# huakunyang/SummerTTS

Measured on AMD Instinct MI355X. Metric: audio samples/sec (acoustic model + vocoder, phoneme ids -> int16 PCM on host), single_speaker_fast-shaped synthetic blob, higher is better.
Workload: dtype f32 (decoder trunk convs AND the reverse flow's WaveNet convs (wn_flow.hip, one-utterance calls): fp32 operands as 2 fp16 terms = 22-23 of their 24 mantissa bits, 3 fp16 MFMA products per fp32 product, f32 accumulation -- measured error in `parity`, same tolerance as the exact-fp32 leg; batches addi

## Files before the change

### include/summertts_hip.h

```cpp
#ifndef SUMMERTTS_HIP_H_
#define SUMMERTTS_HIP_H_

#include <stdint.h>

#ifdef __cplusplus
extern "C" {
#endif

typedef struct sts_engine sts_engine;

enum {
    STS_OK = 0,
    STS_EINVAL = -1,
    STS_EMODEL = -2,
    STS_EDEVICE = -3,
    STS_ESTATE = -4
};

int sts_create(const float* blob, int64_t blob_bytes, int device, sts_engine** out);
void sts_destroy(sts_engine* e);

int sts_speaker_num(const sts_engine* e);

typedef struct sts_model_info {
// ... 61 lines not shown

enum { STS_DBG_ATTN_BLOCK_MIN_WGS = 1,
       STS_DBG_TAIL_FUSED = 14 ,
       STS_DBG_UPS_ROWPH = 15 ,
       STS_DBG_CHAIN_STREAMS = 13 ,
       STS_DBG_H2P = 11 ,
       STS_DBG_H2P_TILE = 12 ,
       STS_DBG_MEMO_CLEAR = 10 ,
       STS_DBG_PCM_DIRECT = 9 ,
       STS_DBG_DDS_TAIL = 8 ,
       STS_DBG_ATTN_REG = 7 ,
       STS_DBG_LAUNCH_AHEAD = 6 ,
       STS_DBG_FLOW_FUSED = 5  };
enum { STS_DBG_STREAM_RETRY_STEP = 16, STS_DBG_STREAM_DIRECT = 17 };
enum { STS_DBG_POISON = 18 };
int sts_debug_set(sts_engine* e, int key, int value);

typedef struct sts_profile {
    float ms_text_encoder, ms_duration, ms_flow, ms_decoder, ms_total_device;
    float ms_decoder_mfma;
    int32_t decoder_mfma_launches;
    double flops_text_encoder, flops_duration, flops_flow, flops_decoder;
    double flops_decoder_mfma;
    double bytes_decoder_min;
    int64_t frames, samples, phonemes;
    double flops_decoder_mfma_executed;
    double bytes_text_encoder, bytes_duration, bytes_flow;
    float ms_sync_wait_host;
    double flops_decoder_bf16_issued;
    int64_t conv_math_fallbacks;
    int32_t conv_math_pinned;
    int32_t launch_ahead;
    int64_t launch_ahead_misses;
    float us_host_setup;
    float us_host_enqueue;
    float us_host_tail;
    int64_t poison_bytes;
} sts_profile;
int sts_set_profiling(sts_engine* e, int enable);
#define STS_ABI_VERSION 13
int sts_abi_version(void);
int sts_build_flags(void);
int sts_get_profile(const sts_engine* e, sts_profile* p);
int sts_get_profile_ex(const sts_engine* e, void* p, int64_t size_bytes);

int sts_debug_conv1d(int device, const float* x, int32_t Cin, int32_t L, const float* w, const float* bias,
                     int32_t Cout, int32_t k, int32_t pad, int32_t dil, int32_t stride_transposed,
                     int32_t depthwise, float in_slope, int32_t in_act, int mode, float** y, int32_t* Lout);

int sts_debug_conv1d_bench(int device, const float* x, int32_t Cin, int32_t L, const float* w, const float* bias,
                           int32_t Cout, int32_t k, int32_t pad, int32_t dil, int32_t stride_transposed,
                           int32_t depthwise, float in_slope, int32_t in_act, int mode, float** y, int32_t* Lout,
                           int32_t iters, float* ms_out);

int sts_debug_conv_h2p(int device, const float* x, int32_t Cin, int32_t L, const float* w, const float* bias, int32_t Cout, int32_t k,
// ... 53 lines not shown
```

### summertts_amd/csrc/capi.hip

```cpp
#include <stdlib.h>
#include <string.h>

#include <algorithm>
#include <new>
#include <string>
#include <vector>

#include "engine.hpp"

using namespace sts;

struct sts_engine { Engine eng; };

static thread_local std::string g_err;
static int set_err(int code, const std::string& s) { g_err = s; return code; }

extern "C" {

const char* sts_last_error(void) { return g_err.c_str(); }
void sts_free(void* p) { free(p); }

int sts_create(const float* blob, int64_t blob_bytes, int device, sts_engine** out) {
    if (!out) return set_err(STS_EINVAL, "sts_create: null out pointer");
    *out = nullptr;
// ... 157 lines not shown
        case STS_DBG_ATTN_BLOCK_MIN_WGS: if (value < 1) return set_err(STS_EINVAL, "threshold must be >= 1"); e->eng.attn_block_min_wgs = value; return STS_OK;
        case STS_DBG_FLOW_FUSED: e->eng.flow_fused = value != 0; return STS_OK;
        case STS_DBG_LAUNCH_AHEAD: if (value < 0 || value > 2) return set_err(STS_EINVAL, "launch_ahead must be 0, 1 or 2"); if ((value == 2) != (e->eng.launch_ahead == 2)) { e->eng.seen_tf_.clear(); e->eng.seen_order_.clear(); } e->eng.launch_ahead = value; return STS_OK;
        case STS_DBG_H2P: e->eng.h2p = value < 0 ? 0 : (value > 4 ? 4 : value); return STS_OK;
        case STS_DBG_H2P_TILE: e->eng.h2p_tile = value; return STS_OK;
        case STS_DBG_CHAIN_STREAMS: e->eng.chain_streams_dbg = value; return STS_OK;
        case STS_DBG_TAIL_FUSED: e->eng.tail_fused = value != 0; return STS_OK;
        case STS_DBG_UPS_ROWPH: e->eng.ups_rowph = value != 0; return STS_OK;
        case STS_DBG_MEMO_CLEAR: e->eng.seen_tf_.clear(); e->eng.seen_order_.clear(); return STS_OK;
        case STS_DBG_ATTN_REG: e->eng.attn_reg = value != 0; return STS_OK;
        case STS_DBG_DDS_TAIL: e->eng.dds_tail = value != 0; return STS_OK;
        case STS_DBG_PCM_DIRECT: e->eng.pcm_direct = value != 0; return STS_OK;
        case STS_DBG_STREAM_RETRY_STEP: e->eng.stream_retry_step = value < 0 ? -1 : value; return STS_OK;
        case STS_DBG_STREAM_DIRECT: e->eng.stream_direct = value != 0; return STS_OK;
        case STS_DBG_POISON: e->eng.poison = (unsigned)value; return STS_OK;
        default: return set_err(STS_EINVAL, "unknown debug key");
    }
}
int sts_set_host_pcm(sts_engine* e, int enable) { if (!e) return set_err(STS_EINVAL, "null engine"); e->eng.host_pcm = enable != 0; return STS_OK; }
int sts_set_profiling(sts_engine* e, int enable) { if (!e) return set_err(STS_EINVAL, "null engine"); e->eng.profiling = enable == 2 ? 2 : (enable != 0 ? 1 : 0); return STS_OK; }

int sts_abi_version(void) { return STS_ABI_VERSION; }

int sts_set_output_rate(sts_engine* e, int32_t rate) {
    if (!e) return set_err(STS_EINVAL, "null engine");
    const int rc = e->eng.set_output_rate(rate);
    return rc == STS_OK ? STS_OK : set_err(rc, e->eng.error());
}
int sts_get_output_rate(const sts_engine* e) {
    if (!e) return set_err(STS_EINVAL, "null engine");
// ... 489 lines not shown
```

### summertts_amd/csrc/conv_bf3.hip

```cpp
#include "conv_bf3_dev.hpp"

namespace sts {

#ifdef STS_TILE_TRACE
int tile_trace_bind_group(long long* buf, unsigned capacity_records);
int tile_trace_bind_resblock(long long* buf, unsigned capacity_records);
int tile_trace_bind_flow(long long* buf, unsigned capacity_records);
int tile_trace_bind_h2p(long long* buf, unsigned capacity_records);
static long long* g_tt_host_buf = nullptr;
extern "C" int sts_debug_tile_trace(long long* buf, unsigned capacity_records) {
    g_tt_host_buf = buf;
    if (buf && hipMemset(buf, 0, 16 * sizeof(long long)) != hipSuccess) return -1;
    if (tile_trace_bind(buf, capacity_records) || tile_trace_bind_group(buf, capacity_records) || tile_trace_bind_resblock(buf, capacity_records) || tile_trace_bind_flow(buf, capacity_records) || tile_trace_bind_h2p(buf, capacity_records)) return -1;
    return 0;
}
extern "C" int sts_debug_tile_trace_count() {
    unsigned n = 0;
    if (!g_tt_host_buf || hipMemcpy(&n, g_tt_host_buf, sizeof(unsigned), hipMemcpyDeviceToHost) != hipSuccess) return -1;
    return (int)n;
}
#endif

static inline void split_host(float x, uint16_t (&p)[3]) {
    uint32_t u; memcpy(&u, &x, 4);
// ... 55 lines not shown
    return bytes;
}

bool conv_bf3_eligible(const ConvArgs& a) {
    if (!a.wb3 || a.depthwise || (a.in_reflect && a.transposed)) return false;
    if (a.Cin != a.Cin_pad || a.Cin_pad % CK != 0 || a.Cout_pad % 32 != 0 || a.Cin < 32) return false;
    if ((double)a.x_ld * 64.0 >= 4.0e9) return false;
    const int first = a.tap_off, last = a.tap_off + (a.ntap - 1) * a.tap_step;
    const int halo = first < last ? last - first : first - last;
    if (halo > MAX_HALO) return false;
    if (a.epi == EPI_GATE && !a.gate_perm) return false;
    if (a.epi == EPI_TANH_PCM || a.kslices > 1) return false;
    return true;
}

template <int MW, int NW, int WM, int WN, int NSUB, int KG = 1, bool H2 = false, bool SUM = false>
static void launch_bf3(const ConvArgs& a, int nphase, hipStream_t st, int pm = 0) {
    constexpr int MT = 32 * MW * WM, NT = 32 * NW * WN;
    pm = pm && a.transposed && (MW == 1 || a.Cout_pad % (32 * MW) == 0);
    const int mt = pm ? (a.Cout_pad * nphase + MT - 1) / MT : (a.Cout_pad + MT - 1) / MT;
    const int nx = (a.max_n + NT - 1) / NT, ny = pm ? mt : mt * nphase;
    if constexpr (SUM) {
        if (a.nsum >= 2) {
            if (a.math == 1) {
                const size_t lds = bf3_lds_bytes<MW, NW, WM, WN, NSUB, KG, 1>();
                hipLaunchKernelGGL((conv_bf3_kernel<MW, NW, WM, WN, NSUB, KG, 1, true>), dim3(mapped_grid(nx, ny, a.B)), dim3(WM * WN * KG * 64), lds, st, a, mt, nx, ny, pm);
            } else {
                const size_t lds = bf3_lds_bytes<MW, NW, WM, WN, NSUB, KG>();
                hipLaunchKernelGGL((conv_bf3_kernel<MW, NW, WM, WN, NSUB, KG, 0, true>), dim3(mapped_grid(nx, ny, a.B)), dim3(WM * WN * KG * 64), lds, st, a, mt, nx, ny, pm);
            }
            return;
        }
    }
    if constexpr (H2) {
        if (a.math == 1) {
            const size_t lds = bf3_lds_bytes<MW, NW, WM, WN, NSUB, KG, 1>();
// ... 13 lines not shown
    const int nphase = bf3_phases(a);
    const int tile = bf3_pick(a);
    const int mt = tile == 4 ? 32 : (tile == 3 ? 64 : 128), nt = tile == 4 ? 256 : 128;
    return (long)((a.max_n + nt - 1) / nt) * ((bf3_phase_rows(a) + mt - 1) / mt) * nphase * a.B;
}

bool conv_bf3_takes_sum(const ConvArgs& a) {
    if (!conv_bf3_eligible(a) || a.in_reflect || a.nsum < 2 || a.nsum > 3 || !a.xs1 || (a.nsum == 3 && !a.xs2)) return false;
    const int nphase = bf3_phases(a);
    const int tile = bf3_pick(a);
    if (tile == 22) return (long)nphase * bf3_phase_rows(a) <= 2 * 128;
    if (tile == 23) return (long)nphase * bf3_phase_rows(a) <= 2 * 64;
    return false;
}

void conv_bf3(const ConvArgs& a, hipStream_t st, int tile) {
    const int nphase = a.rowph ? 1 : bf3_phases(a);
    if (a.max_n <= 0 || a.B <= 0) return;
    if (!bf3_tile_ok(tile) || (a.math == 1 && !h2_tile(tile))) tile = bf3_pick(a);
    if (tile >= 8 && tile < 16 && a.Cin_pad % 32 != 0) tile -= 8;
    if (a.nsum >= 2 && tile != 22 && tile != 23) tile = bf3_pick(a);
    switch (tile) {
        case 20: if (a.Cin_pad % 32 == 0) { launch_bf3<2, 2, 2, 2, 2, 2, true>(a, nphase, st); break; } launch_bf3<2, 2, 2, 2, 1, 1, true>(a, nphase, st); break;
        case 22: launch_bf3<2, 2, 2, 2, 1, 1, true, true>(a, nphase, st, a.rowph ? 0 : 1); break;
        case 23: launch_bf3<1, 2, 2, 2, 1, 1, true, true>(a, nphase, st, a.rowph ? 0 : 1); break;
        case 0: launch_bf3<2, 2, 2, 2, 1, 1, true>(a, nphase, st); break;
        case 3: launch_bf3<2, 2, 1, 2, 1, 1, true>(a, nphase, st); break;
#ifdef STS_EXPERIMENTS
        case 24: if (a.Cin_pad % 32 == 0) { launch_bf3<2, 2, 4, 1, 2, 2, true>(a, nphase, st); break; } launch_bf3<2, 2, 2, 2, 1, 1, true>(a, nphase, st); break;
        case 21: launch_bf3<2, 2, 4, 2, 1>(a, nphase, st, 1); break;
        case 1: launch_bf3<2, 2, 1, 4, 1>(a, nphase, st); break;
        case 2: launch_bf3<2, 2, 2, 4, 1>(a, nphase, st); break;
        case 5: launch_bf3<1, 2, 1, 2, 1>(a, nphase, st); break;
        case 6: launch_bf3<1, 4, 4, 1, 1>(a, nphase, st); break;
        case 7: launch_bf3<1, 4, 2, 1, 1>(a, nphase, st); break;
        case 14: launch_bf3<1, 4, 4, 1, 2>(a, nphase, st); break;
        case 15: launch_bf3<1, 4, 2, 1, 2>(a, nphase, st); break;
        case 8: launch_bf3<2, 2, 2, 2, 2>(a, nphase, st); break;
        case 9: launch_bf3<2, 2, 1, 4, 2>(a, nphase, st); break;
        case 10: launch_bf3<2, 2, 2, 4, 2>(a, nphase, st); break;
        case 11: launch_bf3<2, 2, 1, 2, 2>(a, nphase, st); break;
// ... 9 lines not shown
```

### summertts_amd/csrc/conv_bf3_dev.hpp

```cpp
#pragma once
#include "kernels.hpp"
#include "devmath.hpp"
#include "conv_common.hpp"
#include "knobs.hpp"

#include <stdlib.h>
#include <string.h>

namespace sts {

typedef __bf16 bf16x8 __attribute__((ext_vector_type(8)));
typedef unsigned u32x4 __attribute__((ext_vector_type(4)));

#ifndef STS_EXP
#define STS_EXP 0
#endif
#ifndef STS_VAR
#define STS_VAR 6
#endif
#ifndef STS_H2_AR
#define STS_H2_AR 2
#endif
#ifndef STS_GROUP_RPF
#define STS_GROUP_RPF 0
// ... 113 lines not shown
#pragma unroll
        for (int i = 0; i < MW; i++) p2[i] = __builtin_bit_cast(u32x4, __builtin_bit_cast(f16x8, ac[i][0]) * (_Float16)0.00048828125f);
#ifndef STS_H2_PRODUCTS_FROM
#define STS_H2_PRODUCTS_FROM 0
#endif
#pragma unroll
        for (int p = STS_H2_PRODUCTS_FROM; p < 3; p++)
#pragma unroll
            for (int i = 0; i < MW; i++)
#pragma unroll
                for (int q = 0; q < NW; q++) acc[i][q] = mfma_f16(p == 0 ? p2[i] : ac[i][kProdAh[p]], bc[q][kProdBh[p]], acc[i][q]);
    }
}


template <int MW, int NW, int WM, int WN, int NSUB = 1, int KG = 1, bool NTL = false, int MATH = 0, bool NSUM = false, bool RPF = false>
__device__ __forceinline__ void conv_bf3_body(const ConvArgs& a, const int mtiles, const int bx, const int by, const int b, const int pm = 0, [[maybe_unused]] const int tt_member = 0) {
    static_assert(NSUB % KG == 0 && (KG == 1 || NW % KG == 0), "K groups take whole sub-chunks and whole column tiles");
    constexpr int MT = 32 * MW * WM, NT = 32 * NW * WN, NTW = WM * WN, NWAVE = NTW * KG;
    constexpr int WIN = NT + MAX_HALO;
    constexpr int NSLOT = WIN / 32;
    constexpr int NITEM = NSLOT * NSUB;
    constexpr int SPW = (NITEM + NWAVE - 1) / NWAVE;
    constexpr int NPB = MATH ? 2 : 3;
    constexpr int NPA = MATH ? 2 : 3;
    constexpr unsigned ABLK = NPA * 1024u;
    constexpr int PLANE = WIN * 32, SUB = NPB * PLANE, BUF = NSUB * SUB;
    extern __shared__ __attribute__((aligned(16))) unsigned char smem3[];
#ifdef STS_TILE_TRACE
    long long* tt_rec = tt_open(0, tt_member);
    TT_STAMP(0);
// ... 238 lines not shown
        __syncthreads();
        static_for<0, KG>([&](auto gc) {
            constexpr int g = decltype(gc)::value;
            if (kg == g) {
                f32x16 mine[MW][NW / KG];
                static_for<0, MW>([&](auto ic) {
                    constexpr int i = decltype(ic)::value;
                    static_for<0, NW / KG>([&](auto qc) {
                        constexpr int qq = decltype(qc)::value;
#pragma unroll
                        for (int r = 0; r < 16; r++)
                            mine[i][qq][r] = acc[i][qq * KG + g][r] + red[(size_t)g * REG + (((size_t)(tw * MW + i) * (NW / KG) + qq) * 16 + r) * 64 + lane];
                    });
                });
                static_assert(KG == 1 || NW / KG == 1, "one column tile per group");
                if (wvalid) tile_epilogue<MW, NW / KG>(a, mine, mbase, n0 + wn * NW * 32 + g * 32, l31, half, n_count, out_len, out_base, phase, b);
            }
        });
#ifdef STS_TILE_TRACE
        asm volatile("s_waitcnt vmcnt(0)" ::: "memory");
        TT_STAMP(3);
        TT_CLOSE();
#endif
        return;
    }
    if ((STS_EXP & 32) && acc[0][0][0] != 12345.f) return;
    TT_STAMP(2);
    if constexpr (RPF) {
        if (wvalid) tile_epilogue_pre<MW, NW, NTL>(a, acc, mbase, n0 + wn * NW * 32, l31, half, n_count, out_len, out_base, phase, b, rpre, rpf);
    } else {
        if (wvalid) tile_epilogue<MW, NW, NTL>(a, acc, mbase, n0 + wn * NW * 32, l31, half, n_count, out_len, out_base, phase, b);
    }
#ifdef STS_TILE_TRACE
    asm volatile("s_waitcnt vmcnt(0)" ::: "memory");
    TT_STAMP(3);
    TT_CLOSE();
#endif
}

template <int MW, int NW, int WM, int WN, int NSUB, int KG = 1, int MATH = 0, bool NSUM = false>
__global__ __launch_bounds__(WM* WN * KG * 64) __attribute__((amdgpu_waves_per_eu(MATH ? STS_H2_MINW : 1, MATH ? (MW == 1 && KG == 1 ? STS_MW1_WAVES : STS_H2_WAVES) : 2))) void conv_bf3_kernel(ConvArgs a, int mtiles, int nx, int ny, int pm) {
    const TileId t = map_tile(nx, ny, a.B);
    if (!t.valid) return;
    conv_bf3_body<MW, NW, WM, WN, NSUB, KG, false, MATH, NSUM>(a, mtiles, t.bx, t.by, t.bz, pm);
}

template <int MW, int NW, int WM, int WN, int NSUB, int KG = 1, int MATH = 0>
__global__ __launch_bounds__(WM* WN * KG * 64) __attribute__((amdgpu_waves_per_eu(MATH ? (KG == 1 && MW == 2 && WM == 2 ? STS_GROUP_MINW : STS_H2_MINW) : 1,
                                                                                     MATH ? (KG == 1 && MW == 2 && WM == 2 ? STS_GROUP_WAVES : STS_H2_WAVES) : 2))) void conv_bf3_group_kernel(ConvGroup G, int mtiles, int B, int nx, int ny, int interleave) {
    const TileId t = map_tile(nx, ny, B * G.n);
    if (!t.valid) return;
    int gi, bx, b;
    if (interleave) { const int unit = t.bz * nx + t.bx; gi = unit % G.n; const int rest = unit / G.n; bx = rest % nx; b = rest / nx; }
    else { gi = t.bz / B; bx = t.bx; b = t.bz - gi * B; }
    const ConvArgs* ga = (const ConvArgs*)__builtin_amdgcn_kernarg_segment_ptr();
    conv_bf3_body<MW, NW, WM, WN, NSUB, KG, false, MATH, false, STS_GROUP_RPF && KG == 1 && MATH == 1>(ga[gi], mtiles, bx, t.by, b, 0, gi);
}

constexpr int kNumBf3Tiles = 8;
// ... 32 lines not shown
```

### summertts_amd/csrc/decoder.hip

```cpp
#include "run_ctx.hpp"
#include "knobs.hpp"

#include <math.h>
#include <string.h>
#include <utility>

namespace sts {

static constexpr int MAX_HALO_H2P = 64;

int decoder_halo_frames(const Model& M) {
    double R = M.dec_type == 0 ? (M.conv_post.k - 1) / 2 : (M.conv_post.k - 1) / 2 + 12;
    const int nk = M.n_resk;
    for (int i = M.n_up - 1; i >= 0; i--) {
        double rb = 0;
        for (int j = 0; j < nk; j++) {
            const DResBlock& b = M.rb[(size_t)i * nk + j];
            double r = 0;
            for (size_t d = 0; d < b.c1.size(); d++) r += b.c1[d].dil * (b.c1[d].k - 1) / 2 + b.c2[d].dil * (b.c2[d].k - 1) / 2;
            if (r > rb) rb = r;
        }
        R += rb;
        const DConv& up = M.ups[i];
        R = ceil((R + up.k) / (double)up.stride) + 1;
// ... 47 lines not shown
    StagedBf3,
    StagedMfma
};
static bool is_fused(LayerKind k) { return k == LayerKind::FusedBf3 || k == LayerKind::FusedWino || k == LayerKind::FusedDirect; }

struct LayerArgs {
    ConvGroup G1, G2;
    ResLayerGroup R;
    H2PGroup H1, H2;
    double fl, flw;
};

struct Engine::ResStage {
    Engine& e; const int i, nk, nd0; const DConv& up; const Lvl& l2; const StageBufs b;
    bool grouped = false, per_chain = false, h2p_stage = false;
    int rank[8] = {};
    const float* cur[kMaxGroup] = {};
    ResStage(Engine& e_, int i_, const Lvl& l2_, float* reg, size_t ce)
        : e(e_), i(i_), nk(e_.model.n_resk), nd0(nk > 0 ? (int)e_.model.rb[(size_t)i_ * nk].c1.size() : 0), up(e_.model.ups[i_]), l2(l2_), b{reg, ce, nk} {
        chain_rank(e.model, i, rank);
    }
    const DResBlock& rb(int j) const { return e.model.rb[(size_t)i * nk + j]; }
    hipStream_t aux(int j) const { return e.aux_[rank[j] % kAux]; }
    long fused128_tiles() const { return (long)((l2.max_len + 117) / 118) * l2.nb * nk; }
    void fork() const { (void)hipEventRecord(e.ev_fork_, e.stream); for (int k = 0; k < kAux; k++) (void)hipStreamWaitEvent(e.aux_[k], e.ev_fork_, 0); }
    void join(int n) const { for (int k = 0; k < n; k++) { (void)hipEventRecord(e.ev_join_[k], e.aux_[k]); (void)hipStreamWaitEvent(e.stream, e.ev_join_[k], 0); } }

    bool probe_grouped();
    void plan();
    bool fuse_candidate(int d) const;
// ... 116 lines not shown

void Engine::ResStage::launch(LayerKind k, int d, const LayerArgs& A) const {
    const hipStream_t stream = e.stream;
    static const char* gt = exp_env("STS_GROUP_TILE");
    const int gtile = gt && (int)strlen(gt) > i ? gt[i] - '0' : -1;
    if (is_fused(k)) {
        auto run = [&](const ResLayerGroup& R, hipStream_t st) {
            static const int bv = exp_int("STS_BF3_LAYER_VARIANT", -1);
            if (k == LayerKind::FusedBf3) resblock_bf3(R, st, bv);
            else if (k == LayerKind::FusedWino) resblock_wino(R, st);
            else resblock_layer(R, st);
        };
        if (!per_chain) return run(A.R, stream);
        for (int j = 0; j < nk; j++) { ResLayerGroup R1 = A.R; R1.n = 1; R1.g[0] = A.R.g[j]; run(R1, aux(j)); }
    } else if (k == LayerKind::H2PPair) {
        if (d == 0) split_planes(b.up(), l2.ld, up.Cout, l2.seg, l2.nb, l2.max_len, 0.1f, b.P0(), b.X0(), l2.ld, e.ovf_, stream);
        const int ht = e.h2p_tile < 0 ? -1 : (up.Cout == 128 ? (e.h2p_tile & 0xff) : ((e.h2p_tile >> 8) & 0xff));
        conv_h2p_group(A.H1, stream, ht == 0xff ? -1 : ht);
        conv_h2p_group(A.H2, stream, ht == 0xff ? -1 : ht);
    } else if (per_chain) {
        for (int j = 0; j < nk; j++)
            for (const ConvArgs* ca : {&A.G1.g[j], &A.G2.g[j]}) {
                if (k == LayerKind::StagedBf3 && conv_bf3_eligible(*ca)) conv_bf3(*ca, aux(j), -1);
                else if (conv_mfma_eligible(*ca)) conv_mfma(*ca, aux(j), gtile);
                else conv_generic(*ca, aux(j));
            }
    } else if (k == LayerKind::StagedBf3) {
        static const char* bgt = exp_env("STS_BF3_GROUP_TILE");
        const int bt = bgt && (int)strlen(bgt) > i ? (bgt[i] >= '0' && bgt[i] <= '9' ? bgt[i] - '0' : (bgt[i] >= 'a' && bgt[i] <= 'z' ? bgt[i] - 'a' + 10 : -1)) : -1;
        conv_bf3_group(A.G1, stream, bt);
        conv_bf3_group(A.G2, stream, bt);
// ... 77 lines not shown
    mark(5);
    in_mfma_region_ = true;
    for (int i = 0; i < M.n_up; i++) {
        const DConv& up = M.ups[i];
        const int S2 = S * M.up_rate[i];
        const Lvl l2 = lvF(S2, 0);
        const size_t ce = (size_t)up.Cout * l2.total;
        ResStage st(*this, i, l2, (i & 1) ? bf.regB : bf.regA, ce);
        float* bup = st.b.up();
        ConvOpt ou; ou.in_act = 1; ou.slope = 0.1f;
        {
            static const char* ut = exp_env("STS_UP_TILE");
            if (ut && (int)strlen(ut) > i && ut[i] >= '0' && ut[i] <= '7') ou.tile = ut[i] - '0';
        }
        with_mean(ou);
        conv(up, x, lx, bup, l2, ou);
        mean.n = 0;
        const int nk = st.nk;
        const float* outs[8];
        st.plan();
        if (st.grouped) st.run_grouped(outs); else st.run_forked(outs);
        if (nk == 1) x = outs[0];
        else if (nk <= 3 && !no_sum_fold) { mean.p[0] = outs[0]; mean.p[1] = outs[1]; mean.p[2] = nk > 2 ? outs[2] : nullptr; mean.n = nk; mean.dst = bup; mean.count = (long)ce; x = outs[0]; }
        else { sum_scale(bup, outs, nk, (long)ce, stream); x = bup; }
        S = S2; lx = l2;
    }
    in_mfma_region_ = false;
    mark(6);

    float* wave = record_taps || resampling() || lim_mode != 0 || (loud_mode != 0 && !ss) ? bf.wave : nullptr;
    int16_t* const pcm = bf.pcm_nat;
    const long Ntot = Wtot * hop;
    if (M.dec_type == 0) {
        ConvOpt o; o.in_act = 1; o.slope = 1e-2f; o.epi = EPI_TANH_PCM; o.pcm = pcm; o.aux = wave;
        with_mean(o);
        conv(M.conv_post, x, lx, nullptr, lx, o);
// ... 80 lines not shown
```

### summertts_amd/csrc/engine.hip

```cpp
#include "run_ctx.hpp"
#include <time.h>
#include "knobs.hpp"
#include "../../include/tts_logger.h"

#include <algorithm>
#include <chrono>
#include <math.h>
#include <stdlib.h>
#include <string.h>
#include <thread>

namespace sts {

Engine::~Engine() {
    if (stream) (void)hipStreamSynchronize(stream);
    free_model(model);
    if (arenaT_.base) (void)hipFree(arenaT_.base);
    if (arenaF_.base) (void)hipFree(arenaF_.base);
    if (pinned_) (void)hipHostFree(pinned_);
    if (pinned_pcm_) (void)hipHostFree(pinned_pcm_);
    if (d_rs_table) (void)hipFree(d_rs_table);
    if (loud_host_) (void)hipHostFree(loud_host_);
    if (lim_host_) (void)hipHostFree(lim_host_);
    if (ovf_host_) (void)hipHostFree(ovf_host_);
// ... 134 lines not shown
        double by = 4.0 * ((double)c.Cin * lin.total + (double)c.Cout * lout.total);
        if (o.res || o.epi == EPI_SUB || o.epi == EPI_RESSKIP) by += 4.0 * (double)c.Cout * lout.total;
        bytes_[cur_stage_] += by;
        bytes_w_[cur_stage_] += 4.0 * (double)wfl;
    }
    if (flops) *flops = fl;
    return a;
}

void Engine::conv(const DConv& c, const float* x, const Lvl& lin, float* y, const Lvl& lout, const ConvOpt& o) {
    double fl = 0;
    ConvArgs a = conv_args(c, x, lin, y, lout, o, &fl);
    const bool can_mfma = conv_mode != 1 && conv_mfma_eligible(a);
    const bool use_bf3 = conv_mode == 0 && conv_math != 1 && o.tile < 0 && conv_bf3_eligible(a) &&
                         (in_mfma_region_ || conv_math == 2 || conv_bf3_blocks(a) >= 384);
    if (use_bf3 && c.transposed && ups_rowph && a.epi == EPI_STORE && !a.ubias && (a.math == 1 ? c.wh2r : c.wb3r)) {
        a.wb3 = a.math == 1 ? c.wh2r : c.wb3r;
        a.bias = c.bias ? c.bias_r : nullptr;
        a.Cout = a.Cout_pad = c.Cout_pad * c.stride;
        a.rowph = c.stride;
    }
    if (a.nsum >= 2 && !(use_bf3 ? conv_bf3_takes_sum(a) : (!can_mfma && conv_cout1_takes(a)))) {
        const float* r[3] = {x, o.sum1, o.sum2};
        sum_scale(o.sum_dst, r, a.nsum, o.sum_n, cur_);
        a.x = o.sum_dst; a.xs1 = a.xs2 = nullptr; a.nsum = 0;
    }
    if (use_bf3) {
        if (in_mfma_region_) { mfma_flops_ += fl; bf16_exec_ += products() * fl; mfma_launches_++; }
        static const int bt = exp_int("STS_BF3_TILE", -1);
        conv_bf3(a, cur_, bt);
    } else if (can_mfma) {
// ... 1120 lines not shown
```

### summertts_amd/csrc/engine.hpp

```cpp
#pragma once
#include <hip/hip_runtime.h>

#include <deque>
#include <map>
#include <unordered_map>
#include <string>
#include <vector>

#include "../../include/summertts_hip.h"
#include "kernels.hpp"
#include "model.hpp"

namespace sts {

struct Arena {
    char* base = nullptr; size_t cap = 0, used = 0; bool measuring = false;
    void* alloc(size_t bytes) {
        size_t a = (used + 255) & ~(size_t)255;
        used = a + bytes;
        if (measuring) return nullptr;
        return base + a;
    }
    template <typename T> T* get(size_t count) { return (T*)alloc(count * sizeof(T)); }
};
// ... 1 lines not shown
struct Lvl {
    SegView seg; int nb = 0; int max_len = 0; long total = 0; long ld = 0;
};

struct ConvOpt {
    int in_act = 0; float slope = 0.f; int reflect = 0;
    int epi = EPI_STORE, epi_flag = 0; float epi_scale = 1.f;
    const float* res = nullptr; long res_ld = 0;
    float* aux = nullptr; long aux_ld = 0;
    int16_t* pcm = nullptr;
    const float* ubias = nullptr;
    int pad_l = -1;
    int tile = -1;
    int kslices = 1; long kslice_stride = 0;
    const float* sum1 = nullptr; const float* sum2 = nullptr; int nsum = 0; float* sum_dst = nullptr; long sum_n = 0;
};

struct StreamSpec {
    int chunk_frames; int (*cb)(void* user, const int16_t* pcm, int32_t n_samples, int32_t sample_offset); void* user;
    int (*bcb)(void* user, int32_t utt, const int16_t* pcm, int32_t n_samples, int32_t sample_offset) = nullptr;
    int32_t* delivered = nullptr;
};
int decoder_halo_frames(const Model& M);
struct WinGeom;
inline bool noise_scale_valid(float s) { return s >= 0.f && s <= 3.0e38f; }
inline bool loudness_args_valid(int mode, float target, float peak) {
    return mode >= 0 && mode <= 2 && target >= -70.f && target <= 0.f && peak >= -30.f && peak <= 0.f;
}
void limiter_stats_decode(const unsigned* raw, int B, sts_limiter_stats* out);

// ... 54 lines not shown
    int launch_ahead = 1;
    long ahead_misses = 0;
    static constexpr size_t kMemoEntries = 1024;
    std::unordered_map<unsigned long long, long> seen_tf_; std::deque<unsigned long long> seen_order_;
    bool polite_wait = false;
    struct WaitEst { double us = 0.0; long phonemes = 0; };
    WaitEst wait_est_[2][24];
    void nap_before_wait(int which, long phonemes);
    void note_wait(int which, long phonemes, double waited_us, bool was_ready_at_wake);
    int final_sync(long phonemes);
    int ups_rowph = 1;
    int tail_fused = 1;
    int chain_streams_dbg = -1;
    int h2p = 1;
    int h2p_tile = -1;
    int flow_fused = 1;
    int stream_retry_step = -1;
    int stream_direct = 0;
    unsigned poison = 0;
    int64_t poison_bytes_ = 0;
    hipStream_t stream = nullptr;

private:
    int fail(int code, const std::string& msg) { err_ = msg; return code; }
    bool ensure(Arena& a, size_t bytes);
    bool ensure_pinned(size_t bytes);
    void poison_arena(const Arena& a);
    void poison_host16(void* p, size_t samples);
    void poison_host32(void* p, size_t words);
    ConvArgs conv_args(const DConv& c, const float* x, const Lvl& lin, float* y, const Lvl& lout, const ConvOpt& o, double* flops);
// ... 26 lines not shown
    char* pinned_pcm_ = nullptr; size_t pinned_pcm_cap_ = 0;
    int16_t* pinned_pcm_dev_ = nullptr;
    unsigned* ovf_host_ = nullptr; unsigned* ovf_ = nullptr;
    int* hmap_ = nullptr; int* hmap_dev_ = nullptr; size_t hmap_cap_ = 0;
    unsigned* arrive_ = nullptr; int seq_ = 0;
    float* loud_host_ = nullptr; float* loud_dev_ = nullptr; int loud_cap_ = 0;
    LoudCoef loud_k_{}; int loud_k_rate_ = 0;
    unsigned* lim_host_ = nullptr; int lim_cap_ = 0;
    hipEvent_t ev_[8] = {};
    static constexpr int kAux = 3;
    hipStream_t aux_[kAux] = {};
    hipEvent_t ev_fork_ = nullptr, ev_join_[kAux] = {};
    hipEvent_t ev_setup_ = nullptr;
    hipStream_t cur_ = nullptr;
    bool have_events_ = false;
    int cur_stage_ = 0;
    double flops_[4] = {0, 0, 0, 0};
    double bytes_[4] = {0, 0, 0, 0};
    double bytes_w_[4] = {0, 0, 0, 0};
    double mfma_flops_ = 0, mfma_exec_ = 0, bf16_exec_ = 0, sync_wait_ms_ = 0; int mfma_launches_ = 0; bool in_mfma_region_ = false;
};

}
```

### summertts_amd/csrc/kernels.hpp

```cpp
#pragma once
#include <hip/hip_runtime.h>
#include <stdint.h>

namespace sts {

struct SegView {
    const int* off;
    const int* len;
    int scale;
    int extra;
    int ioff, ilen;
};

enum Epilogue : int {
    EPI_STORE = 0,
    EPI_RESADD = 1,
    EPI_SUB = 3,
    EPI_GATE = 4,
    EPI_RESSKIP = 5,
    EPI_TANH_PCM = 6,
};

struct ConvArgs {
    const float* x; long x_ld;
// ... 10 lines not shown
    int transposed, n_extra;
    int depthwise;
    int in_act; float in_slope;
    int in_reflect;
    int epi, epi_flag; float epi_scale; int H;
    int gate_perm;
    SegView in_seg, out_seg;
    int B, max_n;
    int kslices; long kslice_stride;
    const float* wu; int wino_n3, wino_n2;
    const void* wb3;
    int keep_lo, keep_hi;
    int math; float wscale; unsigned* ovf;
    const float* xs1; const float* xs2; int nsum;
    int rowph;
};

__host__ __device__ inline void wino_split(int k, int* n3, int* n2) { *n2 = (k % 3 == 0) ? 0 : (k % 3 == 2 ? 1 : 2); *n3 = (k - 2 * *n2) / 3; }
void wino_pack(const float* w, long s_out, long s_tap, long s_in, int Cout, int k, int Cin, int Cin_pad, int Cout_pad, float* dst);
bool conv_wino_eligible(const ConvArgs& a);
void conv_wino(const ConvArgs& a, hipStream_t st);

struct LnArgs {
    const float* a; long a_ld;
    const float* b; long b_ld;
    int nb; long b_stride;
    const float* res; long res_ld;
    float* y; long y_ld;
    const float* gamma; const float* beta;
    int C;
// ... 87 lines not shown
    float ws1, ws2;
};
struct ResLayerGroup {
    ResLayerArgs g[kMaxGroup];
    int n, C; long ld; float slope;
    SegView seg; int B; int max_n;
    int math; unsigned* ovf;
};
bool resblock_layer_eligible(const ResLayerGroup& G);
void resblock_layer(const ResLayerGroup& G, hipStream_t st);
bool resblock_wino_eligible(const ResLayerGroup& G);
void resblock_wino(const ResLayerGroup& G, hipStream_t st);
bool conv_group_eligible(const ConvGroup& G);
bool conv_bf3_eligible(const ConvArgs& a);
bool conv_bf3_takes_sum(const ConvArgs& a);
bool conv_cout1_takes(const ConvArgs& a);
void conv_bf3(const ConvArgs& a, hipStream_t st, int tile = -1);
long conv_bf3_blocks(const ConvArgs& a);
bool conv_bf3_group_eligible(const ConvGroup& G);
void conv_bf3_group(const ConvGroup& G, hipStream_t st, int tile = -1);
size_t bf3_pack(const float* wp, int nphase, int ntap, int Cin_pad, int Cout_pad, void* dst, bool perm_k = false, int math = 0, float* wscale = nullptr);
bool resblock_bf3_eligible(const ResLayerGroup& G);
void resblock_bf3(const ResLayerGroup& G, hipStream_t st, int variant = -1);
void conv_mfma_group(const ConvGroup& G, hipStream_t st, int tile = -1);

struct H2PArgs {
    const void* xp; long xp_ld;
    const void* wb; float wscale;
    const float* bias;
    const float* res16; long res_ld;
// ... 105 lines not shown
```

### summertts_amd/csrc/model.hip

```cpp
#include "model.hpp"
#include "kernels.hpp"

#include <hip/hip_runtime.h>
#include <math.h>
#include <string.h>

namespace sts {

namespace {

struct Reader {
    const float* p; int64_t n; int64_t o = 0; bool ok = true;
    int geti() { if (o >= n) { ok = false; return 0; } return (int)p[o++]; }
    const float* take(int64_t cnt) {
        if (cnt < 0 || o + cnt > n) { ok = false; return p; }
        const float* r = p + o; o += cnt; return r;
    }
};

HConv parse_conv(Reader& r) {
    HConv c;
    c.out_ch = r.geti(); c.in_ch = r.geti(); c.k = r.geti(); c.pad = r.geti(); c.dil = r.geti(); c.has_bias = r.geti();
    if (c.out_ch <= 0 || c.in_ch <= 0 || c.k <= 0 || c.out_ch > (1 << 20) || c.in_ch > (1 << 20) || c.k > 4096) { r.ok = false; return c; }
    c.w = r.take((int64_t)c.in_ch * c.k * c.out_ch);
// ... 194 lines not shown
    float* p = st.alloc((bytes + 3) / 4 + 1024, &dptr);
    if (!p) return false;
    bf3_pack(wr.data(), 1, d.J, d.Cin_pad, rows, p, false);
    const size_t hbytes = bf3_pack(nullptr, 1, d.J, d.Cin_pad, rows, nullptr, false, 1);
    const float* hptr = nullptr;
    float* q = st.alloc((hbytes + 3) / 4 + 1024, &hptr);
    if (!q) return false;
    float sc = 1.0f;
    bf3_pack(wr.data(), 1, d.J, d.Cin_pad, rows, q, false, 1, &sc);
    if (sc != d.h2_scale) return true;
    const float* bptr = nullptr;
    float* b = st.alloc((size_t)rows, &bptr);
    if (!b) return false;
    if (d.bias) { const float* bh = st.host.data() + (d.bias - st.dev); for (int r = 0; r < rows; r++) b[r] = bh[r / s]; }
    d.wb3r = dptr; d.wh2r = hptr; d.bias_r = bptr;
    return true;
}

bool pack_h2p(Store& st, DConv& d) {
    if (d.wh2p || d.depthwise || d.transposed || !d.w || d.Cin != d.Cin_pad || d.Cout != d.Cout_pad || d.Cin != d.Cout || d.Cin % 128 != 0) return true;
    const float* hptr = nullptr;
    const size_t hbytes = bf3_pack(nullptr, 1, d.k, d.Cin_pad, d.Cout_pad, nullptr, true, 1);
    float* q = st.alloc((hbytes + 3) / 4 + 2048, &hptr);
    if (!q) return false;
    const float* wh = st.host.data() + (d.w - st.dev);
    float sc = 1.0f;
    bf3_pack(wh, 1, d.k, d.Cin_pad, d.Cout_pad, q, true, 1, &sc);
    d.wh2p = hptr; d.h2_scale = sc;
    return true;
}
// ... 383 lines not shown
```

### summertts_amd/csrc/model.hpp

```cpp
#pragma once
#include <stdint.h>
#include <string>
#include <vector>

namespace sts {

struct HConv {
    int out_ch = 0, in_ch = 0, k = 0, pad = 0, dil = 1, has_bias = 0, stride = 1;
    const float* w = nullptr;
    const float* b = nullptr;
};
struct HLn { int size = 0; const float* g = nullptr; const float* b = nullptr; };

struct DConv {
    int Cin = 0, Cout = 0, Cin_pad = 0, Cout_pad = 0;
    int k = 0, pad = 0, dil = 1;
    int depthwise = 0;
    int transposed = 0, stride = 1, J = 1;
    int gate_perm = 0, H = 0;
    const float* w = nullptr;
    const float* bias = nullptr;
    const float* wc = nullptr;
    const float* bias_rows = nullptr;
    const float* wu = nullptr;
    const void* wb3 = nullptr;
    const void* wb3p = nullptr;
    const void* wh2 = nullptr;
    const void* wh2p = nullptr;
    float h2_scale = 1.0f;
    const void* wb3r = nullptr; const void* wh2r = nullptr; const float* bias_r = nullptr;
    double macs_per_out = 0;
};
struct DLn { int C = 0; const float* g = nullptr; const float* b = nullptr; };

struct PackOpts {
    bool reverse_in = false;
    bool reverse_out = false;
    bool gate = false;
    int gate_H = 0;
    bool gate_blocks = false;
    bool depthwise = false;
    int out_rows = -1;
};

struct DMha { int ch = 0, kc = 0, win = 0, px = 0; const float* relk = nullptr; const float* relv = nullptr; DConv qkv, o; };
// ... 41 lines not shown
```

### summertts_amd/engine.py

```python
from __future__ import annotations

import ctypes as C
import os
import subprocess
from typing import Dict, List, Optional, Sequence

import numpy as np

_HERE = os.path.dirname(os.path.abspath(__file__))
LIB_PATH = os.environ.get("SUMMERTTS_HIP_LIB") or os.path.join(_HERE, "lib", "libsummertts_hip.so")
CSRC = os.path.join(_HERE, "csrc")


def build_library(verbose: bool = False) -> str:
    subprocess.run(["make", "-C", CSRC, "-j8"], check=True, stdout=None if verbose else subprocess.DEVNULL)
    return LIB_PATH


class ModelInfo(C.Structure):
    _fields_ = [("is_multi_speaker", C.c_int32), ("lang_type", C.c_int32), ("dur_pred_type", C.c_int32),
                ("dec_type", C.c_int32), ("vocab", C.c_int32), ("hidden", C.c_int32), ("inter_channels", C.c_int32),
                ("speaker_num", C.c_int32), ("gin_channels", C.c_int32), ("samples_per_frame", C.c_int32),
                ("sample_rate", C.c_int32), ("blob_floats_consumed", C.c_int64)]

# ... 368 lines not shown
        out = np.zeros(n, LIMITER_DTYPE)
        if n:
            rc = self.lib.sts_get_limiter(self.h, out.ctypes.data, n)
            if rc < 0:
                _check(self.lib, rc)
        return out

    def set_conv_math(self, mode):
        m = {"bf16x3": 0, "f32": 1, "bf16x3_all": 2, "f16x2": 3}.get(mode, mode)
        _check(self.lib, self.lib.sts_set_conv_math(self.h, int(m)))

    def set_conv_mode(self, mode: int):
        _check(self.lib, self.lib.sts_set_conv_mode(self.h, mode))

    def debug_set(self, key: str, value: int):
        _check(self.lib, self.lib.sts_debug_set(self.h, {"attn_block_min_wgs": 1, "flow_fused": 5, "launch_ahead": 6, "attn_reg": 7, "dds_tail": 8, "pcm_direct": 9, "memo_clear": 10, "h2p": 11, "h2p_tile": 12, "chain_streams": 13, "tail_fused": 14, "ups_rowph": 15, "stream_retry_step": 16, "stream_direct": 17, "poison": 18}[key], int(value)))

    def set_profiling(self, on):
        _check(self.lib, self.lib.sts_set_profiling(self.h, 2 if on == 2 else (1 if on else 0)))

    def profile(self) -> dict:
        p = Profile()
        _check(self.lib, self.lib.sts_get_profile_ex(self.h, C.byref(p), C.sizeof(p)))
        return p.as_dict()

    def tap(self, name: str) -> np.ndarray:
        ptr = C.POINTER(C.c_float)()
        ch, ln = C.c_int32(), C.c_int64()
        _check(self.lib, self.lib.sts_get_tap(self.h, name.encode(), C.byref(ptr), C.byref(ch), C.byref(ln)))
        a = np.ctypeslib.as_array(ptr, shape=(ch.value, ln.value)).copy()
        self.lib.sts_free(ptr)
# ... 305 lines not shown
```

Measured before the change: 66.37 million.

## Fuse fp16 plane split into transposed upsample conv epilogue

Adds an epilogue variant to the bf3 transposed-conv kernel that writes the upsampled activation directly in the split fp16 hi/lo plane layout used by the following H2P residual stage, plus an fp32 copy. To support this, weights and bias are repacked in a channel-chunked row order. When the fused epilogue runs, the separate split_planes pass is skipped, which removes one full read and write of the upsample output. In exchange it adds a weight layout, more template instances and extra global stores per tile.

After: 66.93 million (median of 4 runs). No clear change (+0.9%).

```diff
diff --git a/include/summertts_hip.h b/include/summertts_hip.h
--- a/include/summertts_hip.h
+++ b/include/summertts_hip.h
@@ -99,6 +99,7 @@
        STS_DBG_FLOW_FUSED = 5  };
 enum { STS_DBG_STREAM_RETRY_STEP = 16, STS_DBG_STREAM_DIRECT = 17 };
 enum { STS_DBG_POISON = 18 };
+enum { STS_DBG_H2P_ENTRY = 19 };
 int sts_debug_set(sts_engine* e, int key, int value);
 
 typedef struct sts_profile {
@@ -123,7 +124,7 @@
     int64_t poison_bytes;
 } sts_profile;
 int sts_set_profiling(sts_engine* e, int enable);
-#define STS_ABI_VERSION 13
+#define STS_ABI_VERSION 14
 int sts_abi_version(void);
 int sts_build_flags(void);
 int sts_get_profile(const sts_engine* e, sts_profile* p);
diff --git a/summertts_amd/csrc/capi.hip b/summertts_amd/csrc/capi.hip
--- a/summertts_amd/csrc/capi.hip
+++ b/summertts_amd/csrc/capi.hip
@@ -195,6 +195,7 @@
         case STS_DBG_STREAM_RETRY_STEP: e->eng.stream_retry_step = value < 0 ? -1 : value; return STS_OK;
         case STS_DBG_STREAM_DIRECT: e->eng.stream_direct = value != 0; return STS_OK;
         case STS_DBG_POISON: e->eng.poison = (unsigned)value; return STS_OK;
+        case STS_DBG_H2P_ENTRY: e->eng.h2p_entry = value != 0; return STS_OK;
         default: return set_err(STS_EINVAL, "unknown debug key");
     }
 }
diff --git a/summertts_amd/csrc/conv_bf3.hip b/summertts_amd/csrc/conv_bf3.hip
--- a/summertts_amd/csrc/conv_bf3.hip
+++ b/summertts_amd/csrc/conv_bf3.hip
@@ -93,12 +93,19 @@
     return true;
 }
 
-template <int MW, int NW, int WM, int WN, int NSUB, int KG = 1, bool H2 = false, bool SUM = false>
+template <int MW, int NW, int WM, int WN, int NSUB, int KG = 1, bool H2 = false, bool SUM = false, bool HP = false>
 static void launch_bf3(const ConvArgs& a, int nphase, hipStream_t st, int pm = 0) {
     constexpr int MT = 32 * MW * WM, NT = 32 * NW * WN;
     pm = pm && a.transposed && (MW == 1 || a.Cout_pad % (32 * MW) == 0);
     const int mt = pm ? (a.Cout_pad * nphase + MT - 1) / MT : (a.Cout_pad + MT - 1) / MT;
     const int nx = (a.max_n + NT - 1) / NT, ny = pm ? mt : mt * nphase;
+    if constexpr (HP) {
+        if (a.hp) {
+            const size_t lds = bf3_lds_bytes<MW, NW, WM, WN, NSUB, KG, 1>();
+            hipLaunchKernelGGL((conv_bf3_kernel<MW, NW, WM, WN, NSUB, KG, 1, false, true>), dim3(mapped_grid(nx, ny, a.B)), dim3(WM * WN * KG * 64), lds, st, a, mt, nx, ny, 0);
+            return;
+        }
+    }
     if constexpr (SUM) {
         if (a.nsum >= 2) {
             if (a.math == 1) {
@@ -142,17 +149,26 @@
     return false;
 }
 
+bool conv_bf3_takes_hp(const ConvArgs& a) {
+    if (!conv_bf3_eligible(a) || !a.hp || !a.hp16 || a.math != 1 || !a.transposed || a.epi != EPI_STORE || a.ubias || a.in_reflect) return false;
+    if ((a.rowph != 2 && a.rowph != 4 && a.rowph != 8) || a.rowph != a.out_stride) return false;
+    if (a.Cout != a.Cout_pad || (a.Cout / a.rowph) % 128 != 0) return false;
+    if ((double)a.hp_ld * 32.0 >= 2.0e9) return false;
+    const int tile = bf3_pick(a);
+    return tile == 0 || tile == 20;
+}
+
 void conv_bf3(const ConvArgs& a, hipStream_t st, int tile) {
     const int nphase = a.rowph ? 1 : bf3_phases(a);
     if (a.max_n <= 0 || a.B <= 0) return;
-    if (!bf3_tile_ok(tile) || (a.math == 1 && !h2_tile(tile))) tile = bf3_pick(a);
+    if (!bf3_tile_ok(tile) || (a.math == 1 && !h2_tile(tile)) || a.hp) tile = bf3_pick(a);
     if (tile >= 8 && tile < 16 && a.Cin_pad % 32 != 0) tile -= 8;
     if (a.nsum >= 2 && tile != 22 && tile != 23) tile = bf3_pick(a);
     switch (tile) {
-        case 20: if (a.Cin_pad % 32 == 0) { launch_bf3<2, 2, 2, 2, 2, 2, true>(a, nphase, st); break; } launch_bf3<2, 2, 2, 2, 1, 1, true>(a, nphase, st); break;
+        case 20: if (a.Cin_pad % 32 == 0) { launch_bf3<2, 2, 2, 2, 2, 2, true, false, true>(a, nphase, st); break; } launch_bf3<2, 2, 2, 2, 1, 1, true, false, true>(a, nphase, st); break;
         case 22: launch_bf3<2, 2, 2, 2, 1, 1, true, true>(a, nphase, st, a.rowph ? 0 : 1); break;
         case 23: launch_bf3<1, 2, 2, 2, 1, 1, true, true>(a, nphase, st, a.rowph ? 0 : 1); break;
-        case 0: launch_bf3<2, 2, 2, 2, 1, 1, true>(a, nphase, st); break;
+        case 0: launch_bf3<2, 2, 2, 2, 1, 1, true, false, true>(a, nphase, st); break;
         case 3: launch_bf3<2, 2, 1, 2, 1, 1, true>(a, nphase, st); break;
 #ifdef STS_EXPERIMENTS
         case 24: if (a.Cin_pad % 32 == 0) { launch_bf3<2, 2, 4, 1, 2, 2, true>(a, nphase, st); break; } launch_bf3<2, 2, 2, 2, 1, 1, true>(a, nphase, st); break;
diff --git a/summertts_amd/csrc/conv_bf3_dev.hpp b/summertts_amd/csrc/conv_bf3_dev.hpp
--- a/summertts_amd/csrc/conv_bf3_dev.hpp
+++ b/summertts_amd/csrc/conv_bf3_dev.hpp
@@ -151,7 +151,60 @@
 }
 
 
-template <int MW, int NW, int WM, int WN, int NSUB = 1, int KG = 1, bool NTL = false, int MATH = 0, bool NSUM = false, bool RPF = false>
+template <int MW, int NW>
+__device__ __forceinline__ void tile_epilogue_h2p(const ConvArgs& a, f32x16 (&acc)[MW][NW], const int mbase, const int ncol0, const int l31, const int half,
+                                                 const int n_count, const int out_len, const size_t out_base) {
+    const int out_off = uni(a.out_off), s = uni(a.out_stride);
+    const int crow = 16 * s;
+    unsigned char* const hp = (unsigned char*)uni((void*)a.hp);
+    float* const hp16 = uni(a.hp16);
+    const size_t ld = (size_t)uni(a.hp_ld);
+    const size_t ps = (size_t)(uni(a.Cout) / s) * ld * 2u;
+    const float* const bias = uni(a.bias);
+    const float slope = a.hp_slope;
+    float amax = 0.f;
+    static_for<0, MW>([&](auto ic) {
+        constexpr int i = decltype(ic)::value;
+        const int row0 = mbase + i * 32;
+        if (row0 < a.Cout) {
+            const int cc = row0 / crow, ph0 = (row0 - cc * crow) >> 4;
+            f32x4u bv[2][2];
+#pragma unroll
+            for (int hh = 0; hh < 2; hh++)
+#pragma unroll
+                for (int u = 0; u < 2; u++)
+                    bv[hh][u] = bias ? *(const f32x4u*)(bias + row0 + 16 * hh + 8 * u + 4 * half) : f32x4u{0.f, 0.f, 0.f, 0.f};
+            static_for<0, NW>([&](auto qc) {
+                constexpr int q = decltype(qc)::value;
+                const int n = ncol0 + q * 32 + l31;
+#pragma unroll
+                for (int hh = 0; hh < 2; hh++) {
+                    const int pos = n * s + out_off + ph0 + hh;
+                    if (n < n_count && pos >= 0 && pos < out_len) {
+                        float v[8], t[8];
+#pragma unroll
+                        for (int e = 0; e < 8; e++) v[e] = acc[i][q][hh * 8 + e] + bv[hh][e >> 2][e & 3];
+                        const size_t unit = (size_t)cc * ld + out_base + (size_t)pos;
+                        float* o = hp16 + (unit * 16 + half * 8);
+                        *(f32x4u*)o = f32x4u{v[0], v[1], v[2], v[3]};
+                        *(f32x4u*)(o + 4) = f32x4u{v[4], v[5], v[6], v[7]};
+#pragma unroll
+                        for (int e = 0; e < 8; e++) t[e] = __builtin_fmaxf(v[e], v[e] * slope);
+                        u32x4 ph, pl;
+                        split8h(t, ph, pl, amax);
+                        unsigned char* d = hp + (unit * 32 + half * 16);
+                        *(u32x4*)d = ph;
+                        *(u32x4*)(d + ps) = pl;
+                    }
+                }
+                __builtin_amdgcn_sched_barrier(0);
+            });
+        }
+    });
+    if (amax > kH2Limit && a.ovf) *a.ovf = 1u;
+}
+
+template <int MW, int NW, int WM, int WN, int NSUB = 1, int KG = 1, bool NTL = false, int MATH = 0, bool NSUM = false, bool RPF = false, bool HP = false>
 __device__ __forceinline__ void conv_bf3_body(const ConvArgs& a, const int mtiles, const int bx, const int by, const int b, const int pm = 0, [[maybe_unused]] const int tt_member = 0) {
     static_assert(NSUB % KG == 0 && (KG == 1 || NW % KG == 0), "K groups take whole sub-chunks and whole column tiles");
     constexpr int MT = 32 * MW * WM, NT = 32 * NW * WN, NTW = WM * WN, NWAVE = NTW * KG;
@@ -420,7 +473,8 @@
                     });
                 });
                 static_assert(KG == 1 || NW / KG == 1, "one column tile per group");
-                if (wvalid) tile_epilogue<MW, NW / KG>(a, mine, mbase, n0 + wn * NW * 32 + g * 32, l31, half, n_count, out_len, out_base, phase, b);
+                if constexpr (HP) { if (wvalid) tile_epilogue_h2p<MW, NW / KG>(a, mine, mbase, n0 + wn * NW * 32 + g * 32, l31, half, n_count, out_len, out_base); }
+                else if (wvalid) tile_epilogue<MW, NW / KG>(a, mine, mbase, n0 + wn * NW * 32 + g * 32, l31, half, n_count, out_len, out_base, phase, b);
             }
         });
 #ifdef STS_TILE_TRACE
@@ -432,7 +486,10 @@
     }
     if ((STS_EXP & 32) && acc[0][0][0] != 12345.f) return;
     TT_STAMP(2);
-    if constexpr (RPF) {
+    if constexpr (HP) {
+        static_assert(MATH == 1 && !RPF, "the pre-split epilogue belongs to the two-term fp16 arithmetic");
+        if (wvalid) tile_epilogue_h2p<MW, NW>(a, acc, mbase, n0 + wn * NW * 32, l31, half, n_count, out_len, out_base);
+    } else if constexpr (RPF) {
         if (wvalid) tile_epilogue_pre<MW, NW, NTL>(a, acc, mbase, n0 + wn * NW * 32, l31, half, n_count, out_len, out_base, phase, b, rpre, rpf);
     } else {
         if (wvalid) tile_epilogue<MW, NW, NTL>(a, acc, mbase, n0 + wn * NW * 32, l31, half, n_count, out_len, out_base, phase, b);
@@ -444,11 +501,11 @@
 #endif
 }
 
-template <int MW, int NW, int WM, int WN, int NSUB, int KG = 1, int MATH = 0, bool NSUM = false>
+template <int MW, int NW, int WM, int WN, int NSUB, int KG = 1, int MATH = 0, bool NSUM = false, bool HP = false>
 __global__ __launch_bounds__(WM* WN * KG * 64) __attribute__((amdgpu_waves_per_eu(MATH ? STS_H2_MINW : 1, MATH ? (MW == 1 && KG == 1 ? STS_MW1_WAVES : STS_H2_WAVES) : 2))) void conv_bf3_kernel(ConvArgs a, int mtiles, int nx, int ny, int pm) {
     const TileId t = map_tile(nx, ny, a.B);
     if (!t.valid) return;
-    conv_bf3_body<MW, NW, WM, WN, NSUB, KG, false, MATH, NSUM>(a, mtiles, t.bx, t.by, t.bz, pm);
+    conv_bf3_body<MW, NW, WM, WN, NSUB, KG, false, MATH, NSUM, false, HP>(a, mtiles, t.bx, t.by, t.bz, pm);
 }
 
 template <int MW, int NW, int WM, int WN, int NSUB, int KG = 1, int MATH = 0>
diff --git a/summertts_amd/csrc/decoder.hip b/summertts_amd/csrc/decoder.hip
--- a/summertts_amd/csrc/decoder.hip
+++ b/summertts_amd/csrc/decoder.hip
@@ -2,6 +2,7 @@
 #include "knobs.hpp"
 
 #include <math.h>
+#include <stdio.h>
 #include <string.h>
 #include <utility>
 
@@ -85,6 +86,7 @@
 struct Engine::ResStage {
     Engine& e; const int i, nk, nd0; const DConv& up; const Lvl& l2; const StageBufs b;
     bool grouped = false, per_chain = false, h2p_stage = false;
+    bool entry_split = true;
     int rank[8] = {};
     const float* cur[kMaxGroup] = {};
     ResStage(Engine& e_, int i_, const Lvl& l2_, float* reg, size_t ce)
@@ -231,7 +233,7 @@
         if (!per_chain) return run(A.R, stream);
         for (int j = 0; j < nk; j++) { ResLayerGroup R1 = A.R; R1.n = 1; R1.g[0] = A.R.g[j]; run(R1, aux(j)); }
     } else if (k == LayerKind::H2PPair) {
-        if (d == 0) split_planes(b.up(), l2.ld, up.Cout, l2.seg, l2.nb, l2.max_len, 0.1f, b.P0(), b.X0(), l2.ld, e.ovf_, stream);
+        if (d == 0 && entry_split) split_planes(b.up(), l2.ld, up.Cout, l2.seg, l2.nb, l2.max_len, 0.1f, b.P0(), b.X0(), l2.ld, e.ovf_, stream);
         const int ht = e.h2p_tile < 0 ? -1 : (up.Cout == 128 ? (e.h2p_tile & 0xff) : ((e.h2p_tile >> 8) & 0xff));
         conv_h2p_group(A.H1, stream, ht == 0xff ? -1 : ht);
         conv_h2p_group(A.H2, stream, ht == 0xff ? -1 : ht);
@@ -339,12 +341,20 @@
             if (ut && (int)strlen(ut) > i && ut[i] >= '0' && ut[i] <= '7') ou.tile = ut[i] - '0';
         }
         with_mean(ou);
+        st.plan();
+        if (st.h2p_stage && h2p_entry) { ou.hp = st.b.P0(); ou.hp16 = st.b.X0(); ou.hp_slope = 0.1f; }
         conv(up, x, lx, bup, l2, ou);
+        st.entry_split = !conv_wrote_hp_;
         mean.n = 0;
         const int nk = st.nk;
         const float* outs[8];
-        st.plan();
         if (st.grouped) st.run_grouped(outs); else st.run_forked(outs);
+        if (record_taps && st.h2p_stage) {
+            char nm[32];
+            snprintf(nm, sizeof(nm), "dec%d_planes", i); tap(nm, st.b.P0(), 1, (long)ce, (long)ce);
+            snprintf(nm, sizeof(nm), "dec%d_x16", i); tap(nm, st.b.X0(), 1, (long)ce, (long)ce);
+            snprintf(nm, sizeof(nm), "dec%d_up", i); tap(nm, bup, 1, (long)ce, (long)ce);
+        }
         if (nk == 1) x = outs[0];
         else if (nk <= 3 && !no_sum_fold) { mean.p[0] = outs[0]; mean.p[1] = outs[1]; mean.p[2] = nk > 2 ? outs[2] : nullptr; mean.n = nk; mean.dst = bup; mean.count = (long)ce; x = outs[0]; }
         else { sum_scale(bup, outs, nk, (long)ce, stream); x = bup; }
diff --git a/summertts_amd/csrc/engine.hip b/summertts_amd/csrc/engine.hip
--- a/summertts_amd/csrc/engine.hip
+++ b/summertts_amd/csrc/engine.hip
@@ -172,7 +172,15 @@
     const bool can_mfma = conv_mode != 1 && conv_mfma_eligible(a);
     const bool use_bf3 = conv_mode == 0 && conv_math != 1 && o.tile < 0 && conv_bf3_eligible(a) &&
                          (in_mfma_region_ || conv_math == 2 || conv_bf3_blocks(a) >= 384);
-    if (use_bf3 && c.transposed && ups_rowph && a.epi == EPI_STORE && !a.ubias && (a.math == 1 ? c.wh2r : c.wb3r)) {
+    conv_wrote_hp_ = false;
+    if (o.hp && o.hp16 && use_bf3 && c.transposed && a.math == 1 && c.wh2c && a.epi == EPI_STORE && !a.ubias) {
+        ConvArgs h = a;
+        h.wb3 = c.wh2c; h.bias = c.bias ? c.bias_c : nullptr;
+        h.Cout = h.Cout_pad = c.Cout_pad * c.stride; h.rowph = c.stride;
+        h.hp = o.hp; h.hp16 = o.hp16; h.hp_ld = lout.ld; h.hp_slope = o.hp_slope;
+        if (conv_bf3_takes_hp(h)) { a = h; conv_wrote_hp_ = true; }
+    }
+    if (!conv_wrote_hp_ && use_bf3 && c.transposed && ups_rowph && a.epi == EPI_STORE && !a.ubias && (a.math == 1 ? c.wh2r : c.wb3r)) {
         a.wb3 = a.math == 1 ? c.wh2r : c.wb3r;
         a.bias = c.bias ? c.bias_r : nullptr;
         a.Cout = a.Cout_pad = c.Cout_pad * c.stride;
diff --git a/summertts_amd/csrc/engine.hpp b/summertts_amd/csrc/engine.hpp
--- a/summertts_amd/csrc/engine.hpp
+++ b/summertts_amd/csrc/engine.hpp
@@ -39,6 +39,7 @@
     int tile = -1;
     int kslices = 1; long kslice_stride = 0;
     const float* sum1 = nullptr; const float* sum2 = nullptr; int nsum = 0; float* sum_dst = nullptr; long sum_n = 0;
+    void* hp = nullptr; float* hp16 = nullptr; float hp_slope = 1.f;
 };
 
 struct StreamSpec {
@@ -123,6 +124,7 @@
     int chain_streams_dbg = -1;
     int h2p = 1;
     int h2p_tile = -1;
+    int h2p_entry = 1;
     int flow_fused = 1;
     int stream_retry_step = -1;
     int stream_direct = 0;
@@ -179,6 +181,7 @@
     hipEvent_t ev_setup_ = nullptr;
     hipStream_t cur_ = nullptr;
     bool have_events_ = false;
+    bool conv_wrote_hp_ = false;
     int cur_stage_ = 0;
     double flops_[4] = {0, 0, 0, 0};
     double bytes_[4] = {0, 0, 0, 0};
diff --git a/summertts_amd/csrc/kernels.hpp b/summertts_amd/csrc/kernels.hpp
--- a/summertts_amd/csrc/kernels.hpp
+++ b/summertts_amd/csrc/kernels.hpp
@@ -48,6 +48,7 @@
     int math; float wscale; unsigned* ovf;
     const float* xs1; const float* xs2; int nsum;
     int rowph;
+    void* hp; float* hp16; long hp_ld; float hp_slope;
 };
 
 __host__ __device__ inline void wino_split(int k, int* n3, int* n2) { *n2 = (k % 3 == 0) ? 0 : (k % 3 == 2 ? 1 : 2); *n3 = (k - 2 * *n2) / 3; }
@@ -165,6 +166,7 @@
 bool conv_group_eligible(const ConvGroup& G);
 bool conv_bf3_eligible(const ConvArgs& a);
 bool conv_bf3_takes_sum(const ConvArgs& a);
+bool conv_bf3_takes_hp(const ConvArgs& a);
 bool conv_cout1_takes(const ConvArgs& a);
 void conv_bf3(const ConvArgs& a, hipStream_t st, int tile = -1);
 long conv_bf3_blocks(const ConvArgs& a);
diff --git a/summertts_amd/csrc/model.hip b/summertts_amd/csrc/model.hip
--- a/summertts_amd/csrc/model.hip
+++ b/summertts_amd/csrc/model.hip
@@ -232,6 +232,26 @@
     if (!b) return false;
     if (d.bias) { const float* bh = st.host.data() + (d.bias - st.dev); for (int r = 0; r < rows; r++) b[r] = bh[r / s]; }
     d.wb3r = dptr; d.wh2r = hptr; d.bias_r = bptr;
+    if (d.Cout % 128 == 0) {
+        auto row_of = [&](int co, int ph) { return (co / 16) * 16 * s + ph * 16 + co % 16; };
+        for (int ph = 0; ph < s; ph++)
+            for (int j = 0; j < d.J; j++)
+                for (int ci = 0; ci < d.Cin_pad; ci++) {
+                    const float* src = wh + (((size_t)ph * d.J + j) * d.Cin_pad + ci) * d.Cout_pad;
+                    float* dst = wr.data() + ((size_t)j * d.Cin_pad + ci) * rows;
+                    for (int co = 0; co < d.Cout_pad; co++) dst[row_of(co, ph)] = src[co];
+                }
+        const float* cptr = nullptr;
+        float* qc = st.alloc((hbytes + 3) / 4 + 1024, &cptr);
+        if (!qc) return false;
+        float sc2 = 1.0f;
+        bf3_pack(wr.data(), 1, d.J, d.Cin_pad, rows, qc, false, 1, &sc2);
+        const float* bcptr = nullptr;
+        float* bc = st.alloc((size_t)rows, &bcptr);
+        if (!bc) return false;
+        if (d.bias) { const float* bh = st.host.data() + (d.bias - st.dev); for (int co = 0; co < d.Cout_pad; co++) for (int ph = 0; ph < s; ph++) bc[row_of(co, ph)] = bh[co]; }
+        if (sc2 == d.h2_scale) { d.wh2c = cptr; d.bias_c = bcptr; }
+    }
     return true;
 }
 
diff --git a/summertts_amd/csrc/model.hpp b/summertts_amd/csrc/model.hpp
--- a/summertts_amd/csrc/model.hpp
+++ b/summertts_amd/csrc/model.hpp
@@ -29,6 +29,7 @@
     const void* wh2p = nullptr;
     float h2_scale = 1.0f;
     const void* wb3r = nullptr; const void* wh2r = nullptr; const float* bias_r = nullptr;
+    const void* wh2c = nullptr; const float* bias_c = nullptr;
     double macs_per_out = 0;
 };
 struct DLn { int C = 0; const float* g = nullptr; const float* b = nullptr; };
diff --git a/summertts_amd/engine.py b/summertts_amd/engine.py
--- a/summertts_amd/engine.py
+++ b/summertts_amd/engine.py
@@ -406,7 +406,7 @@
         _check(self.lib, self.lib.sts_set_conv_mode(self.h, mode))
 
     def debug_set(self, key: str, value: int):
-        _check(self.lib, self.lib.sts_debug_set(self.h, {"attn_block_min_wgs": 1, "flow_fused": 5, "launch_ahead": 6, "attn_reg": 7, "dds_tail": 8, "pcm_direct": 9, "memo_clear": 10, "h2p": 11, "h2p_tile": 12, "chain_streams": 13, "tail_fused": 14, "ups_rowph": 15, "stream_retry_step": 16, "stream_direct": 17, "poison": 18}[key], int(value)))
+        _check(self.lib, self.lib.sts_debug_set(self.h, {"attn_block_min_wgs": 1, "flow_fused": 5, "launch_ahead": 6, "attn_reg": 7, "dds_tail": 8, "pcm_direct": 9, "memo_clear": 10, "h2p": 11, "h2p_tile": 12, "chain_streams": 13, "tail_fused": 14, "ups_rowph": 15, "stream_retry_step": 16, "stream_direct": 17, "poison": 18, "h2p_entry": 19}[key], int(value)))
 
     def set_profiling(self, on):
         _check(self.lib, self.lib.sts_set_profiling(self.h, 2 if on == 2 else (1 if on else 0)))
```
